# meijieru/AtomNAS

Hardware: AMD Instinct MI355X
Metric: images/sec (whole node) AtomNAS-C supernet 224x224 bs256/GPU (higher is better)
Workload: dtype bf16; 1 GPU; atomnas_c_supernet full training step (fwd + CE-smooth/L2/L1 + bwd + grad all-reduce + RMSprop + EMA), 224x224; per_gpu_batch=256, global_batch=256, parallelism=dp1, hip_graph=True

## Files before the change

atomnas_amd/csrc/pwconv.hip:

```cpp
#include "pwconv.h"

namespace atomnas {

template <typename T, int MODE, int NCG>
__global__ __launch_bounds__(256) void k_gemm_nt(Operand A, const T* __restrict__ Wp, int ldw, Epilogue ep, long M, int N, int K,
                                                 int Kpad) {
  using MM = Mma<T>;
  constexpr int E = MM::EPL;
  constexpr int KS = 4 * E;
  constexpr int SWD = 64 * NCG;
  extern __shared__ float s_stat[];

  const int tid = threadIdx.x;
  const int lane = tid & 63;
  const int wave = tid >> 6;
  const int q = lane >> 4, j = lane & 15;
  const int wrow = 16 * (j >> 2) + (j & 3);
  const bool do_stats = ep.stats != nullptr && ep.stat_mode != STAT_NONE;
  float* sw = s_stat + wave * 2 * SWD;

  if (do_stats) {
    for (int i = tid; i < 8 * SWD; i += 256) s_stat[i] = 0.f;
    __syncthreads();
  }

  const long mtiles = (M + 15) / 16;
  const int ngroups = (N + SWD - 1) / SWD;
  const int grp = blockIdx.x % ngroups, rs = blockIdx.x / ngroups, R = gridDim.x / ngroups;
  const int nc0 = grp * SWD;
  for (long mt = (long)rs * 4 + wave; mt < mtiles; mt += (long)R * 4) {
    const long m0 = mt * 16;
    const long row = m0 + j;
    const bool rowvalid = row < M;
    {
      f32x4 acc[NCG][4];
#pragma unroll
      for (int g = 0; g < NCG; ++g)
#pragma unroll
        for (int t = 0; t < 4; ++t) acc[g][t] = f32x4{0.f, 0.f, 0.f, 0.f};

#pragma unroll 2
      for (int k0 = 0; k0 < Kpad; k0 += KS) {
        const int k = k0 + q * E;
        float av[E];
        load_pro<T, MODE>(A, row, rowvalid, k, K, av);
        const typename MM::frag af = MM::pack(av);
#pragma unroll
        for (int g = 0; g < NCG; ++g) {
          const int nc = nc0 + 64 * g;
          if (nc < N) {
#pragma unroll
            for (int t = 0; t < 4; ++t) {
              const typename MM::frag wf = MM::raw(Wp + (long)(nc + wrow + 4 * t) * ldw + k);
              acc[g][t] = MM::mma(wf, af, acc[g][t]);
            }
          }
        }
      }

#pragma unroll
      for (int g = 0; g < NCG; ++g) {
        if (nc0 + 64 * g >= N) continue;
        nt_epilogue<T>(ep, acc[g], row, rowvalid, nc0 + 64 * g + 16 * q, N, do_stats, sw, SWD, 64 * g + 16 * q, j);
      }
    }
  }

  if (do_stats) nt_flush_stats(ep, s_stat, SWD, nc0, N, rs, R, tid);
}


typedef __attribute__((ext_vector_type(4))) unsigned u32x4;
typedef __attribute__((ext_vector_type(2))) unsigned u32x2;

template <int MODE, int KST, int NT = 0>
__global__ __launch_bounds__(256) void k_gemm_nt_small(Operand A, const bf16_t* __restrict__ Wp, int ldw, Epilogue ep, long M, int N, int K) {
  using T = bf16_t;
  using MM = Mma<T>;
  constexpr int SWD = 64;
  constexpr int WT = NT > 0 ? NT : 4;
  extern __shared__ float s_stat[];
  const int tid = threadIdx.x;
  const int lane = tid & 63, wave = tid >> 6;
  const int q = lane >> 4, j = lane & 15;
  const int wrow = NT > 0 ? j : 16 * (j >> 2) + (j & 3);
  const bool do_stats = ep.stats != nullptr && ep.stat_mode != STAT_NONE;
  if (do_stats) {
    for (int i = tid; i < 8 * SWD; i += 256) s_stat[i] = 0.f;
    __syncthreads();
  }
  bf16x8 wf[KST][WT];
  float p1[KST][8], p2[KST][8], p3[KST][8];
#pragma unroll
  for (int ks = 0; ks < KST; ++ks) {
    const int k = ks * 32 + 8 * q;
#pragma unroll
    for (int t = 0; t < WT; ++t) wf[ks][t] = MM::raw(Wp + (long)(wrow + (NT > 0 ? 16 : 4) * t) * ldw + k);
#pragma unroll
    for (int e = 0; e < 8; ++e) p1[ks][e] = p2[ks][e] = p3[ks][e] = 0.f;
    if constexpr (MODE != PRO_NONE) {
      if (k < K) {
        VecIO<float, 8>::load(A.c1 + k, p1[ks]);
        VecIO<float, 8>::load(A.c2 + k, p2[ks]);
        if constexpr (MODE == PRO_BNBWD) VecIO<float, 8>::load(A.c3 + k, p3[ks]);
      }
    }
  }
  struct Raw { bf16x8 a, x; };
  Raw nx[KST];
  const long mtiles = (M + 15) / 16;
  const long stride = (long)gridDim.x * 4;
  auto fetch = [&](long mt) {
    const long row = mt * 16 + j;
#pragma unroll
    for (int ks = 0; ks < KST; ++ks) {
      const int k = ks * 32 + 8 * q;
      bf16x8 z;
#pragma unroll
      for (int e = 0; e < 8; ++e) z[e] = (bf16_t)0.f;
      nx[ks].a = z;
      nx[ks].x = z;
      if (row < M && k < K) {
        nx[ks].a = *reinterpret_cast<const bf16x8*>(reinterpret_cast<const T*>(A.p1) + lay_off(row, k, A.ld1, A.ss1));
        if constexpr (MODE == PRO_BNBWD)
          nx[ks].x = *reinterpret_cast<const bf16x8*>(reinterpret_cast<const T*>(A.p2) + lay_off(row, k, A.ld2, A.ss2));
      }
    }
  };
  float s1[16], s2[16];
#pragma unroll
  for (int i = 0; i < 16; ++i) s1[i] = s2[i] = 0.f;
  float e_bias[WT][4], e_zs[WT][4], e_zh[WT][4];
  const Act e_act = act_of(ep.mask);
  if constexpr (NT > 0) {
#pragma unroll
    for (int t = 0; t < NT; ++t)
#pragma unroll
      for (int r = 0; r < 4; ++r) {
        const int n = 16 * t + 4 * q + r;
        e_bias[t][r] = (ep.bias && n < N) ? ep.bias[n] : 0.f;
        e_zs[t][r] = (ep.mask && n < N) ? ep.zscale[n] : 0.f;
        e_zh[t][r] = (ep.mask && n < N) ? ep.zshift[n] : 0.f;
      }
  }

  long mt = (long)blockIdx.x * 4 + wave;
  if (mt < mtiles) fetch(mt);
  for (; mt < mtiles; mt += stride) {
    Raw cur[KST];
#pragma unroll
    for (int ks = 0; ks < KST; ++ks) cur[ks] = nx[ks];
    if (mt + stride < mtiles) fetch(mt + stride);
    const long row = mt * 16 + j;
    const bool rowvalid = row < M;
    f32x4 acc[WT];
#pragma unroll
    for (int t = 0; t < WT; ++t) acc[t] = f32x4{0.f, 0.f, 0.f, 0.f};
#pragma unroll
    for (int ks = 0; ks < KST; ++ks) {
      const int k = ks * 32 + 8 * q;
      float v[8];
#pragma unroll
      for (int e = 0; e < 8; ++e) {
        const float a = (float)cur[ks].a[e];
        if constexpr (MODE == PRO_NONE) v[e] = a;
        else if constexpr (MODE == PRO_BNRELU) v[e] = a * p1[ks][e] + p2[ks][e];
        else v[e] = p1[ks][e] * a + p2[ks][e] * (float)cur[ks].x[e] + p3[ks][e];
      }
      if constexpr (MODE == PRO_BNRELU) act_apply_v<8>(v, act_of(A.relu));
#pragma unroll
      for (int e = 0; e < 8; ++e)
        if (!rowvalid || k + e >= K) v[e] = 0.f;
      const bf16x8 af = MM::pack(v);
#pragma unroll
      for (int t = 0; t < WT; ++t) acc[t] = MM::mma(wf[ks][t], af, acc[t]);
    }
    if constexpr (NT > 0) {
#pragma unroll
      for (int t = 0; t < NT; ++t) {
        const int c0 = 16 * t + 4 * q;
        float c[4], zv[4] = {0.f, 0.f, 0.f, 0.f};
#pragma unroll
        for (int r = 0; r < 4; ++r) c[r] = 0.f;
        if (rowvalid && c0 < N) {
#pragma unroll
          for (int r = 0; r < 4; ++r) c[r] = acc[t][r] + e_bias[t][r];
          if (ep.add) {
            const bf16x4 ad = *reinterpret_cast<const bf16x4*>(reinterpret_cast<const T*>(ep.add) + row * ep.ldadd + c0);
#pragma unroll
            for (int r = 0; r < 4; ++r) c[r] += (float)ad[r];
          }
          if (ep.z) {
            const bf16x4 zb = *reinterpret_cast<const bf16x4*>(reinterpret_cast<const T*>(ep.z) + lay_off(row, c0, ep.ldz, ep.zss));
#pragma unroll
            for (int r = 0; r < 4; ++r) zv[r] = (float)zb[r];
            if (ep.mask) {
              float a4[4];
#pragma unroll
              for (int r = 0; r < 4; ++r) a4[r] = zv[r] * e_zs[t][r] + e_zh[t][r];
              act_bwd_v<4>(c, a4, e_act);
            }
          }
          bf16x4 ob;
#pragma unroll
          for (int r = 0; r < 4; ++r) ob[r] = (bf16_t)c[r];
          u32x2 bits = __builtin_bit_cast(u32x2, ob);
          asm volatile("" : "+v"(bits));
          const f32x2 lo = bf16_pair_f32(bits[0]), hi = bf16_pair_f32(bits[1]);
          c[0] = lo[0]; c[1] = lo[1]; c[2] = hi[0]; c[3] = hi[1];
          *reinterpret_cast<u32x2*>(reinterpret_cast<T*>(ep.c) + lay_off(row, c0, ep.ldc, ep.css)) = bits;
        }
        if (do_stats) {
#pragma unroll
          for (int r = 0; r < 4; ++r) {
            s1[4 * t + r] += c[r];
            s2[4 * t + r] += (ep.stat_mode == STAT_SQ) ? c[r] * c[r] : c[r] * zv[r];
          }
        }
      }
    } else {
      float c[16], zv[16];
      nt_epilogue_core<T>(ep, acc, row, rowvalid, 16 * q, N, c, zv);
      if (do_stats) {
#pragma unroll
        for (int i = 0; i < 16; ++i) {
          s1[i] += c[i];
// ... 1391 lines not shown
    }
    ATOMNAS_RING_STAGE_END();
    islot = islot + 1 == DEPTH ? 0 : islot + 1;
    if (++ic == nchunk) { ic = 0; ++ib; }
  };

  const unsigned tr_lane = (unsigned)(((8 * q + (j >> 2)) * 16 + 4 * (j & 3)) * 2);
  auto tr_frag = [&](unsigned sub_addr) {
    const unsigned a0 = sub_addr + tr_lane;
    bf16x4 lo, hi;
    asm volatile("ds_read_b64_tr_b16 %0, %1" : "=v"(lo) : "v"(a0) : "memory");
    asm volatile("ds_read_b64_tr_b16 %0, %1 offset:128" : "=v"(hi) : "v"(a0) : "memory");
    return TrFrag{lo, hi};
  };

  f32x4 racc[NCH][UT];
#pragma unroll
  for (int c = 0; c < NCH; ++c)
#pragma unroll
    for (int t = 0; t < UT; ++t) racc[c][t] = f32x4{0.f, 0.f, 0.f, 0.f};

#pragma unroll
  for (int s = 0; s < DEPTH - 1; ++s) issue_next();
  int slot = 0;
  const unsigned row_off = (unsigned)(((wave & 1) * 16 + j) * 32);
  for (long n = 0; n < nb; ++n) {
    const long rb = rs + n * R;
    const long row = rb * 64 + wave * 16 + j;
    f32x4 acc[UT];
#pragma unroll
    for (int t = 0; t < UT; ++t) acc[t] = f32x4{0.f, 0.f, 0.f, 0.f};
    bf16x8 xa[2][UT];
#pragma unroll
    for (int c = 0; c < NCH; ++c) {
      if (c < nchunk) {
        asm volatile("s_waitcnt vmcnt(%0)" ::"n"((DEPTH - 2) * 2) : "memory");
        __syncthreads();
        issue_next();
        const unsigned base = lds_st + (unsigned)slot * STAGE_B;
        if (c == 0) {
          const unsigned xb = lds_x + (unsigned)(n & 1) * XT_B;
          TrFrag xf[2][UT];
#pragma unroll
          for (int k2 = 0; k2 < 2; ++k2)
#pragma unroll
            for (int t = 0; t < UT; ++t) xf[k2][t] = tr_frag(xb + (unsigned)(k2 * UT + t) * 1024u);
          asm volatile("s_waitcnt lgkmcnt(0)" ::: "memory");
          __builtin_amdgcn_sched_barrier(0);
#pragma unroll
          for (int k2 = 0; k2 < 2; ++k2) {
            const long rows_left = M - (rb * 64 + 32 * k2);
#pragma unroll
            for (int t = 0; t < UT; ++t) {
              xa[k2][t] = __builtin_shufflevector(xf[k2][t].lo, xf[k2][t].hi, 0, 1, 2, 3, 4, 5, 6, 7);
              if (rows_left < 32) {
#pragma unroll
                for (int e = 0; e < 8; ++e)
                  if (8 * q + e >= rows_left) xa[k2][t][e] = (bf16_t)0.f;
              }
            }
          }
        }
        TrFrag hf[2];
#pragma unroll
        for (int k2 = 0; k2 < 2; ++k2) hf[k2] = tr_frag(base + (unsigned)(4 * k2 + wave) * 1024u);
        bf16x8 hb[2];
#pragma unroll
        for (int ks = 0; ks < 2; ++ks) {
          const unsigned a = base + (unsigned)(4 * (wave >> 1) + 2 * ks + (q >> 1)) * 1024u + row_off + (unsigned)(q & 1) * 16u;
          asm volatile("ds_read_b128 %0, %1" : "=v"(hb[ks]) : "v"(a) : "memory");
        }
        asm volatile("s_waitcnt lgkmcnt(0)" ::: "memory");
        __builtin_amdgcn_sched_barrier(0);
#pragma unroll
        for (int ks = 0; ks < 2; ++ks)
#pragma unroll
          for (int t = 0; t < UT; ++t) {
            const bf16x8 wf = *reinterpret_cast<const bf16x8*>(s_w + (16 * t + j) * KP + 64 * c + 32 * ks + 8 * q);
            acc[t] = MM::mma(wf, hb[ks], acc[t]);
          }
#pragma unroll
        for (int k2 = 0; k2 < 2; ++k2) {
          const bf16x8 hv = __builtin_shufflevector(hf[k2].lo, hf[k2].hi, 0, 1, 2, 3, 4, 5, 6, 7);
#pragma unroll
          for (int t = 0; t < UT; ++t) racc[c][t] = MM::mma(xa[k2][t], hv, racc[c][t]);
        }
        slot = slot + 1 == DEPTH ? 0 : slot + 1;
      }
    }
    const unsigned xrow = lds_x + (unsigned)(n & 1) * XT_B + (unsigned)((wave >> 1) * UT) * 1024u + row_off;
    if (mpk) {
#pragma unroll
      for (int ks = 0; ks < MKS; ++ks) {
        bf16x8 xv;
#pragma unroll
        for (int e = 0; e < 8; ++e) xv[e] = (bf16_t)0.f;
        const int ct = 2 * ks + (q >> 1);
        if (ct < UT) {
          const unsigned a = xrow + (unsigned)ct * 1024u + (unsigned)(q & 1) * 16u;
          asm volatile("ds_read_b128 %0, %1\n\ts_waitcnt lgkmcnt(0)" : "=v"(xv) : "v"(a) : "memory");
        }
#pragma unroll
        for (int t = 0; t < UT; ++t) acc[t] = MM::mma(mf[ks][t], xv, acc[t]);
      }
    }
#pragma unroll
    for (int t = 0; t < UT; ++t) {
      const int c0 = 16 * t + 4 * q;
      bf16x4 av;
#pragma unroll
      for (int r = 0; r < 4; ++r) av[r] = (bf16_t)0.f;
      if (add) {
        const unsigned a = lds_a + (unsigned)(n & 1) * XT_B + (unsigned)((wave >> 1) * UT + t) * 1024u + row_off + (unsigned)(8 * q);
        asm volatile("ds_read_b64 %0, %1\n\ts_waitcnt lgkmcnt(0)" : "=v"(av) : "v"(a) : "memory");
      }
      if (row < M && c0 < N) {
        bf16x4 o;
#pragma unroll
        for (int r = 0; r < 4; ++r) o[r] = (bf16_t)(acc[t][r] + vbv[t][r] + (float)av[r]);
        *reinterpret_cast<bf16x4*>(gx + row * ldgx + c0) = o;
      }
    }
  }
  asm volatile("s_waitcnt vmcnt(0)" ::: "memory");

#pragma unroll
  for (int c = 0; c < NCH; ++c) {
    const int vc = c * 64 + 16 * wave + j;
    if (c < nchunk && vc < K) {
      const float cv = c1[vc];
#pragma unroll
      for (int t = 0; t < UT; ++t)
#pragma unroll
        for (int r = 0; r < 4; ++r) {
          const int uc = 16 * t + 4 * q + r;
          if (uc < N) ws[((long)rs * N + uc) * K + vc] = racc[c][t][r] * cv;
        }
    }
  }
}

struct NtArgs {
  int mode; Operand A;
  const void* Wp; int ldw;
  Epilogue ep;
  long M; int N, K;
  hipStream_t st;
  bool stats;
};
static NtArgs nt_args(int mode, const Operand& A, const void* Wp, int ldw, const Epilogue& ep, long M, int N, int K, hipStream_t st) {
  return NtArgs{mode, A, Wp, ldw, ep, M, N, K, st, ep.stats != nullptr && ep.stat_mode != STAT_NONE};
}

struct PwEnv { int st, sw, swg; long swg_maxm; int small_narrow, xb_stream; };
static const PwEnv& pw_env() {
  static const PwEnv e = {
      getenv("ATOMNAS_NT_ST") ? atoi(getenv("ATOMNAS_NT_ST")) : 1,
      getenv("ATOMNAS_NT_SW") ? atoi(getenv("ATOMNAS_NT_SW")) : 1,
      getenv("ATOMNAS_NT_SWG") ? atoi(getenv("ATOMNAS_NT_SWG")) : 1,
      getenv("ATOMNAS_NT_SWG_MAXM") ? atol(getenv("ATOMNAS_NT_SWG_MAXM")) : 262144,
      getenv("ATOMNAS_NT_SMALL_NARROW") ? atoi(getenv("ATOMNAS_NT_SMALL_NARROW")) : 1,
      getenv("ATOMNAS_XB_STREAM") ? atoi(getenv("ATOMNAS_XB_STREAM")) : 1,
  };
  return e;
}

template <typename KernelT>
static long row_slots(KernelT kern, int threads, size_t lds, int ngroups, long row_blocks, long cap) {
  long R = (long)num_cus() * resident_per_cu(kern, threads, lds) / ngroups;
  if (R > row_blocks) R = row_blocks;
  if (cap > 0 && R > cap) R = cap;
  return R < 1 ? 1 : R;
}
static long stat_cap(const NtArgs& a) { return a.stats ? a.ep.stat_rows : 0; }

template <typename F> static auto for_mode(int mode, F&& f) {
  if (mode == PRO_NONE) return f(IC<PRO_NONE>{});
  if (mode == PRO_BNRELU) return f(IC<PRO_BNRELU>{});
  return f(IC<PRO_BNBWD>{});
}

struct NtSwPlan { int ut, nch, depth; size_t lds; };
constexpr int SW_MAXN = 48, SW_MINK = 97, SW_MAXK = 448;
constexpr long SW_MINM = 16384;
#define SW_INSTANCES(X) X(1, 5) X(1, 7) X(2, 5) X(2, 7) X(3, 5) X(3, 7)

static bool nt_sw_plan(const NtArgs& a, NtSwPlan& p) {
  const Epilogue& ep = a.ep;
  if (!pw_env().sw || a.mode != PRO_BNRELU || a.A.ss1 <= 0 || a.N > SW_MAXN || a.N % 8 != 0 || a.K > SW_MAXK || a.K < SW_MINK ||
      a.M < SW_MINM || ep.out_f32 || ep.css != 0 || ep.add || ep.z || ep.mask || ep.bias || (a.stats && ep.stat_mode != STAT_SQ))
    return false;
  p.ut = (a.N + 15) / 16;
  p.nch = (a.K + 63) / 64 <= 5 ? 5 : 7;
  const size_t fixed = (size_t)16 * p.ut * (p.nch * 64 + 8) * sizeof(bf16_t) + (size_t)2 * p.nch * 64 * sizeof(float) +
                       (size_t)4 * 2 * 16 * p.ut * sizeof(float);
  p.depth = 2 * (fixed + 4 * 8192) + 4096 <= max_lds_bytes() ? 4 : 3;
  p.lds = fixed + (size_t)p.depth * 8192;
  return 2 * p.lds + 2048 <= max_lds_bytes();
}
template <typename KernelT>
static int nt_sw_run(const char* what, KernelT kern, int waves, size_t lds, const NtArgs& a) {
  const long R = row_slots(kern, waves * 64, lds, 1, (a.M + waves * 16 - 1) / (waves * 16), stat_cap(a));
  hipLaunchKernelGGL(kern, dim3((unsigned)R), dim3(waves * 64), lds, a.st, (const bf16_t*)a.A.p1, a.A.ss1, a.A.c1, a.A.c2, a.A.relu,
                     (const bf16_t*)a.Wp, a.ldw, (bf16_t*)a.ep.c, a.ep.ldc, a.stats ? a.ep.stats : nullptr, a.ep.stat_rows, a.M, a.N, a.K);
  return check_launch(what);
}
static int nt_sw_launch(const NtSwPlan& p, const NtArgs& a) {
#define X(UT, NCH) \
  if (p.ut == UT && p.nch == NCH) return nt_sw_run("gemm_nt_sw", p.depth == 4 ? k_gemm_nt_sw<UT, NCH, 4> : k_gemm_nt_sw<UT, NCH, 3>, 4, p.lds, a);
  SW_INSTANCES(X)
#undef X
  return 1;
}

struct NtSwgPlan { int ut; bool wide; size_t lds; };
constexpr int SWG_MAXN = 320, SWG_MINK = 256, SWG_DEPTH = 3;
constexpr long SWG_MINM = 8192;

static bool nt_swg_plan(const NtArgs& a, NtSwgPlan& p) {
  const Epilogue& ep = a.ep;
  if (!pw_env().swg || a.mode != PRO_BNRELU || a.A.ss1 <= 0 || a.N % 8 != 0 || a.N > SWG_MAXN || a.K < SWG_MINK || a.K % 4 != 0 ||
      a.M < SWG_MINM || a.M > pw_env().swg_maxm || a.ldw < 64 || a.ldw % 8 != 0 || ep.out_f32 || ep.css != 0 || ep.add || ep.z || ep.mask ||
      ep.bias || (a.stats && ep.stat_mode != STAT_SQ) || !a.A.c1 || !a.A.c2)
    return false;
  p.ut = (a.N + 15) / 16;
  if (p.ut != 3 && p.ut != 5 && p.ut != 6 && p.ut != 12 && p.ut != 20) return false;
  p.wide = (a.M + 127) / 128 >= num_cus() && p.ut <= 6;
  const int nwv = p.wide ? 8 : 4;
  p.lds = (size_t)nwv * 2 * 16 * p.ut * sizeof(float) + (size_t)SWG_DEPTH * (2 * nwv + 2 * p.ut + 1) * 1024;
  return p.lds <= max_lds_bytes();
}
static int nt_swg_launch(const NtSwgPlan& p, const NtArgs& a) {
#define X(UT, WGPC, NWV) return nt_sw_run("gemm_nt_swg", k_gemm_nt_swg<UT, SWG_DEPTH, WGPC, NWV>, NWV, p.lds, a);
  if (p.wide) {
    if (p.ut == 3) X(3, 1, 8)
    if (p.ut == 5) X(5, 1, 8)
    X(6, 1, 8)
  }
  if (p.ut == 3) X(3, 2, 4)
  if (p.ut == 5) X(5, 2, 4)
  if (p.ut == 6) X(6, 2, 4)
  if (p.ut == 12) X(12, 1, 4)
  X(20, 1, 4)
#undef X
}

struct NtStPlan { int kind, ksteps; };
constexpr int ST_MAXK = 192, ST_MINN = 96;
constexpr long ST_MINM = 1024;

static int nt_st_kind(const NtArgs& a) {
  const Operand& A = a.A;
  const Epilogue& ep = a.ep;
  const long M = a.M, N = a.N, K = a.K;
  if (!pw_env().st || a.mode != PRO_NONE || (K & 7) || ep.bias || ep.add || ep.out_f32) return 0;
  if (ep.stats != nullptr && ep.stat_mode == STAT_NONE) return 0;
  if (a.stats && ((M + 15) / 16 + ep.stat_rows - 1) / ep.stat_rows > 4096) return 0;
  const long a_bytes = A.ss1 ? ((long)((K + 15) / 16 - 1) * A.ss1 + M * 16) * 2 : M * (long)A.ld1 * 2;
  if (a_bytes >= (1L << 31)) return 0;
  if (ep.css ? (3 * ep.css + M * 16) * 2 >= (1L << 31) : ((N & 7) || (long)ep.ldc * 2 * 16 * 4096 >= (1L << 31))) return 0;
  if (!ep.z) return (!a.stats || ep.stat_mode == STAT_SQ) ? ST_FWD : 0;
  if (!ep.mask || (a.stats && ep.stat_mode != STAT_Z)) return 0;
  if (ep.zss ? (3 * ep.zss + M * 16) * 2 >= (1L << 31) : ((N & 7) || (long)ep.ldz * 2 * 16 * 4096 >= (1L << 31))) return 0;
  return ST_MASK;
}
static bool nt_st_plan(const NtArgs& a, NtStPlan& p) {
  if (a.K > ST_MAXK || a.N < 2 * a.K || a.N < ST_MINN || a.M < ST_MINM) return false;
  const int ks = (a.K + 31) / 32;
  p.ksteps = ks <= 3 ? ks : 6;
  p.kind = nt_st_kind(a);
  return p.kind != 0;
}
static long st_tiles_per_item(long mtiles, long wchunks, long waves, long min_tpi, long max_parts) {
  long tpi = (mtiles * wchunks + waves - 1) / waves;
  if (tpi < 8) tpi = 8;
  if (tpi < min_tpi) tpi = min_tpi;
  long max_ranges = waves / wchunks > 0 ? waves / wchunks : 1;
  if (max_parts > 0 && max_ranges > max_parts) max_ranges = max_parts;
  if ((mtiles + tpi - 1) / tpi > max_ranges) tpi = (mtiles + max_ranges - 1) / max_ranges;
  return tpi;
}
template <int KSTEPS, int EPK, bool SH, int BT>
static int nt_st_launch_as(const NtArgs& a) {
  using Cfg = StCfg<KSTEPS, EPK>;
  const Epilogue& ep = a.ep;
  const int nchunks = (a.N + 63) / 64;
  const long mtiles = (a.M + 15) / 16;
  const long min_tpi = ep.stats ? (mtiles + ep.stat_rows - 1) / ep.stat_rows : 1;
  auto kern = k_gemm_nt_st<KSTEPS, EPK, Cfg::PD, BT, Cfg::WPE, 0, SH>;
  const size_t lds = (size_t)(SH ? 2 : 4) * BT * KSTEPS * 1024 +
                     (EPK == ST_FWD ? 0 : (size_t)4 * (16 + 64) * PB_RP * sizeof(bf16_t) + 4 * 128 * sizeof(float));
  const long waves = (long)num_cus() * resident_per_cu(kern, 256, lds) * 4;
  const long wchunks = SH ? (long)((nchunks + 3) / 4) * 4 : nchunks;
  long tiles_per_item = st_tiles_per_item(mtiles, wchunks, waves, min_tpi, 0);
  if (tiles_per_item > 4096) tiles_per_item = 4096;
  const long nrg = (mtiles + tiles_per_item - 1) / tiles_per_item;
  const long blocks = SH ? nrg * ((nchunks + 3) / 4) : (nrg * nchunks + 3) / 4;
  hipLaunchKernelGGL(kern, dim3((unsigned)blocks), dim3(256), lds, a.st, a.A, (const bf16_t*)a.Wp, a.ldw, ep, a.M, a.N, a.K, nchunks,
                     (int)tiles_per_item, (float*)nullptr);
  return check_launch("gemm_nt_st");
}
static int nt_st_launch(const NtStPlan& p, const NtArgs& a) {
  auto go = [&](auto ks, auto epk) {
    constexpr int KSTEPS = decltype(ks)::value, EPK = decltype(epk)::value;
    using Cfg = StCfg<KSTEPS, EPK>;
    const int nchunks = (a.N + 63) / 64;
    if (Cfg::SH && ((nchunks + 3) / 4 * 4 - nchunks) * 20 <= nchunks) return nt_st_launch_as<KSTEPS, EPK, Cfg::SH, Cfg::BT>(a);
    return nt_st_launch_as<KSTEPS, EPK, false, Cfg::BTP>(a);
  };
  auto kind = [&](auto ks) { return p.kind == ST_FWD ? go(ks, IC<ST_FWD>{}) : go(ks, IC<ST_MASK>{}); };
  return p.ksteps == 1 ? kind(IC<1>{}) : p.ksteps == 2 ? kind(IC<2>{}) : p.ksteps == 3 ? kind(IC<3>{}) : kind(IC<6>{});
}

struct NtSmallPlan { int kst, ntile; };
constexpr int SMALL_MAXN = 64, SMALL_MAXK = 64;
constexpr long SMALL_MINM = 65536;

static bool nt_small_plan(const NtArgs& a, NtSmallPlan& p) {
  if (a.N > SMALL_MAXN || a.K > SMALL_MAXK || a.M < SMALL_MINM) return false;
  p.kst = a.K <= 32 ? 1 : 2;
  p.ntile = (pw_env().small_narrow && !a.ep.out_f32 && a.N % 4 == 0) ? (a.N <= 16 ? 1 : a.N <= 32 ? 2 : 4) : 0;
  return true;
}
static int nt_small_launch(const NtSmallPlan& p, const NtArgs& a) {
  auto go = [&](auto mode, auto kst) {
    constexpr int MODE = decltype(mode)::value, KST = decltype(kst)::value;
    auto kern = p.ntile == 1 ? k_gemm_nt_small<MODE, KST, 1> : p.ntile == 2 ? k_gemm_nt_small<MODE, KST, 2>
              : p.ntile == 4 ? k_gemm_nt_small<MODE, KST, 4> : k_gemm_nt_small<MODE, KST, 0>;
    const size_t lds = a.stats ? (size_t)8 * 64 * sizeof(float) : 0;
    const long R = row_slots(kern, 256, lds, 1, (a.M + 63) / 64, stat_cap(a));
    hipLaunchKernelGGL(kern, dim3((unsigned)R), dim3(256), lds, a.st, a.A, (const bf16_t*)a.Wp, a.ldw, a.ep, a.M, a.N, a.K);
  };
  for_mode(a.mode, [&](auto mode) { p.kst == 1 ? go(mode, IC<1>{}) : go(mode, IC<2>{}); });
  return check_launch("gemm_nt_small");
}

struct NtWsPlan { int ncg, rt; };
constexpr int WS_MINK = 97;
constexpr long WS_MINM = 4096;
constexpr long WS_RT2_MINM = 100000;

static bool nt_ws_plan(const NtArgs& a, NtWsPlan& p) {
  if (a.K < WS_MINK || a.M < WS_MINM) return false;
  p.ncg = a.N > 64 ? 2 : 1;
  p.rt = (a.mode == PRO_BNBWD && a.M >= WS_RT2_MINM) ? 2 : 1;
  return true;
}
template <int MODE, int NCG, int RT>
static void nt_ws_launch_as(const NtArgs& a) {
  auto kern = k_gemm_nt_ws<MODE, NCG, RT>;
  const int ngroups = (a.N + 64 * NCG - 1) / (64 * NCG);
  const size_t lds = (size_t)2 * 64 * NCG * WS_WP * sizeof(bf16_t) + 2 * 3 * WS_KC * sizeof(float) +
                     (a.stats ? (size_t)8 * 64 * NCG * sizeof(float) : 0);
  const long R = row_slots(kern, 256, lds, ngroups, (a.M + 64 * RT - 1) / (64 * RT), stat_cap(a));
  const int wrows = (a.N + 63) / 64 * 64;
  hipLaunchKernelGGL(kern, dim3((unsigned)(R * ngroups)), dim3(256), lds, a.st, a.A, (const bf16_t*)a.Wp, a.ldw, wrows, a.ep, a.M, a.N, a.K);
}
static int nt_ws_launch(const NtWsPlan& p, const NtArgs& a) {
  for_mode(a.mode, [&](auto mode) {
    constexpr int MODE = decltype(mode)::value;
    if constexpr (MODE == PRO_BNBWD) {
      if (p.rt == 2) return p.ncg == 2 ? nt_ws_launch_as<MODE, 2, 2>(a) : nt_ws_launch_as<MODE, 1, 2>(a);
    }
    return p.ncg == 2 ? nt_ws_launch_as<MODE, 2, 1>(a) : nt_ws_launch_as<MODE, 1, 1>(a);
  });
  return check_launch("gemm_nt_ws");
}

struct NtGenericPlan { int ncg; };
static bool nt_generic_plan(const NtArgs& a, NtGenericPlan& p) {
  p.ncg = a.N > 64 ? 2 : 1;
  return true;
}
template <typename T>
static int nt_generic_launch(const NtGenericPlan& p, const NtArgs& a) {
  constexpr int KS = 4 * Mma<T>::EPL;
  const int Kpad = (a.K + KS - 1) / KS * KS;
  auto go = [&](auto mode, auto ncg) {
    constexpr int NCG = decltype(ncg)::value;
    auto kern = k_gemm_nt<T, decltype(mode)::value, NCG>;
    const int ngroups = (a.N + 64 * NCG - 1) / (64 * NCG);
    const size_t lds = a.stats ? (size_t)8 * 64 * NCG * sizeof(float) : 0;
    const long R = row_slots(kern, 256, lds, ngroups, (a.M + 63) / 64, stat_cap(a));
    hipLaunchKernelGGL(kern, dim3((unsigned)(R * ngroups)), dim3(256), lds, a.st, a.A, (const T*)a.Wp, a.ldw, a.ep, a.M, a.N, a.K, Kpad);
  };
  for_mode(a.mode, [&](auto mode) { p.ncg == 2 ? go(mode, IC<2>{}) : go(mode, IC<1>{}); });
  return check_launch("gemm_nt");
}

template <typename T>
static int launch_nt(const NtArgs& a) {
  if constexpr (sizeof(T) == 2) {
    NtSwPlan sw;
    if (nt_sw_plan(a, sw)) return nt_sw_launch(sw, a);
    NtSwgPlan swg;
    if (nt_swg_plan(a, swg)) return nt_swg_launch(swg, a);
    NtStPlan st;
    if (nt_st_plan(a, st)) return nt_st_launch(st, a);
    NtSmallPlan small;
    if (nt_small_plan(a, small)) return nt_small_launch(small, a);
    NtWsPlan ws;
    if (nt_ws_plan(a, ws)) return nt_ws_launch(ws, a);
  }
  NtGenericPlan g;
  nt_generic_plan(a, g);
  return nt_generic_launch<T>(g, a);
}

static NtArgs project_bwd_args(const void* g, int ldg, const void* wpt, int ldw, const void* z, int ldz, long z_ss, const float* zscale,
                               const float* zshift, int act, void* gh, int ldgh, long gh_ss, float* stats, int stat_rows, long M, int oup,
                               int hid, hipStream_t st) {
  const Operand A{g, ldg, nullptr, 0, 0, 0, nullptr, nullptr, nullptr, 0};
  const Epilogue ep{gh, ldgh, 0, nullptr, 0, z, ldz, gh_ss, z_ss, zscale, zshift, act, nullptr, stats, STAT_Z, stat_rows};
  return nt_args(PRO_NONE, A, wpt, ldw, ep, M, hid, oup, st);
}
template <int KSTEPS, int UT>
static int launch_project_bwd_st(const NtArgs& a, float* dwp, long si, long sj, float* ws, long ws_floats) {
  using Cfg = StCfg<KSTEPS, ST_PBWD>;
  const long M = a.M;
  const int N = a.N, K = a.K;
  const int nchunks = (N + 63) / 64;
  const long mtiles = (M + 15) / 16;
  auto kern = k_gemm_nt_st<KSTEPS, ST_PBWD, Cfg::PD, Cfg::BT, Cfg::WPE, UT, false>;
  const size_t lds = (size_t)4 * Cfg::BT * KSTEPS * 1024 + (size_t)4 * (16 * UT + 64) * PB_RP * sizeof(bf16_t) + 4 * 128 * sizeof(float);
  const long waves = (long)num_cus() * resident_per_cu(kern, 256, lds) * 4;
  const long max_parts = ws_floats / ((long)K * N);
  ATOMNAS_REQUIRE(max_parts >= 1, "project_bwd: workspace too small for one partial (%ld floats)", (long)K * N);
  const long tiles_per_item = st_tiles_per_item(mtiles, nchunks, waves, (mtiles + a.ep.stat_rows - 1) / a.ep.stat_rows, max_parts);
  ATOMNAS_REQUIRE(tiles_per_item <= 4096, "project_bwd: %ld row tiles per work item (workspace / statistics rows too small for M=%ld)", tiles_per_item, M);
  const long nranges = (mtiles + tiles_per_item - 1) / tiles_per_item;
  const long items = nranges * nchunks;
  hipLaunchKernelGGL(kern, dim3((unsigned)((items + 3) / 4)), dim3(256), lds, a.st, a.A, (const bf16_t*)a.Wp, a.ldw, a.ep, M, N, K, nchunks,
                     (int)tiles_per_item, ws);
  if (int rc = check_launch("project_bwd_st")) return rc;
  return reduce_parts(ws, (long)K * N, (int)nranges, (long)K * N, dwp, N, si, sj, a.st);
}

#define XB_INSTANCES(X) X(1, 5) X(1, 7) X(1, 12) X(2, 5) X(2, 7) X(3, 5)
static inline int xb_nch(int HT) {
  const int n = (HT + WS_KC - 1) / WS_KC;
  return n <= 5 ? 5 : (n <= 7 ? 7 : (n <= 12 ? 12 : 0));
}
static bool xb_has_instance(int inp, int hid) {
  const int ut = (inp + 15) / 16, nch = xb_nch(hid);
#define X(UTV, NCHV) if (ut == UTV && nch == NCHV) return true;
  XB_INSTANCES(X)
#undef X
  return false;
}
struct XbArgs {
  const bf16_t* h; int ldh; long hss; const float* c1;
  const bf16_t* x; int ldx; const bf16_t* W; int ldw; const bf16_t* add; int ldadd; bf16_t* gx; int ldgx;
  const bf16_t* mpk; int ldm; const float* vb;
  float *dwe, *ws; long ws_floats; long M; int N, K; hipStream_t st;
};
template <typename KernelT, typename L>
static int xb_run(const char* what, const XbArgs& a, KernelT kern, size_t lds, L&& launch) {
  const long max_parts = a.ws_floats / ((long)a.N * a.K);
  ATOMNAS_REQUIRE(max_parts >= 1, "expand_bwd: workspace too small for one partial (%ld floats)", (long)a.N * a.K);
  const long R = row_slots(kern, 256, lds, 1, (a.M + 63) / 64, max_parts);
  launch((unsigned)R);
  if (int rc = check_launch(what)) return rc;
  return reduce_parts(a.ws, (long)a.N * a.K, (int)R, (long)a.N * a.K, a.dwe, a.K, 1, a.N, a.st);
}

struct XbStreamPlan { int depth; size_t lds; };
static bool xb_stream_plan(const XbArgs& a, XbStreamPlan& p) {
  if (!pw_env().xb_stream || a.hss <= 0 || a.M < 64 || a.ldx < 8 || (a.add && a.ldadd < 8)) return false;
  if ((a.K + 63) / 64 < 3) return false;
  const int ut = (a.N + 15) / 16, nch = xb_nch(a.K);
  const size_t fixed = (size_t)16 * ut * (nch * 64 + 8) * sizeof(bf16_t) + (size_t)4 * 2 * ut * 1024;
  p.depth = 2 * (fixed + 4 * 8192) + 4096 <= max_lds_bytes() ? 4 : 3;
  p.lds = fixed + (size_t)p.depth * 8192;
  return p.lds <= max_lds_bytes();
}
template <int UT, int NCH>
static int xb_stream_launch(const XbStreamPlan& p, const XbArgs& a) {
  static_assert(4 * UT * NCH <= XB_MINB2_LIMIT, "expand backward instance with too many accumulator registers");
  auto kern = p.depth == 4 ? k_expand_bwd_s<UT, NCH, 4> : k_expand_bwd_s<UT, NCH, 3>;
  return xb_run("expand_bwd(stream)", a, kern, p.lds, [&](unsigned R) {
    hipLaunchKernelGGL(kern, dim3(R), dim3(256), p.lds, a.st, a.h, a.hss, a.c1, a.W, a.ldw, a.x, a.ldx, a.add, a.ldadd, a.gx, a.ldgx, a.mpk,
                       a.ldm, a.vb, a.ws, a.M, a.N, a.K);
  });
}
template <int UT, int NCH>
static int xb_launch(const XbArgs& a) {
  static_assert(4 * UT * NCH <= XB_MINB2_LIMIT, "expand backward instance with too many accumulator registers");
  auto kern = k_expand_bwd<UT, NCH>;
  const size_t lds = (size_t)2 * 64 * WS_WP * sizeof(bf16_t) + 2 * 3 * WS_KC * sizeof(float) + (size_t)2 * 64 * XB_DP * sizeof(bf16_t) +
                     (size_t)16 * UT * XB_DP * sizeof(bf16_t);
  const Operand A{a.h, a.ldh, nullptr, 0, a.hss, 0, a.c1, a.c1, a.c1, 0};
  const Epilogue ep{a.gx, a.ldgx, 0, a.add, a.ldadd, nullptr, 0, 0, 0, nullptr, nullptr, 0, a.vb, nullptr, STAT_NONE, 0};
  const int wrows = (a.N + 63) / 64 * 64;
  return xb_run("expand_bwd", a, kern, lds, [&](unsigned R) {
    hipLaunchKernelGGL(kern, dim3(R), dim3(256), lds, a.st, A, a.W, a.ldw, wrows, a.x, a.ldx, ep, a.ws, a.M, a.N, a.K, a.mpk, a.ldm);
  });
}
static int launch_expand_bwd(const XbArgs& a) {
  const int ut = (a.N + 15) / 16, nch = xb_nch(a.K);
  XbStreamPlan sp;
  const bool stream = xb_stream_plan(a, sp);
#define X(UTV, NCHV) if (ut == UTV && nch == NCHV) return stream ? xb_stream_launch<UTV, NCHV>(sp, a) : xb_launch<UTV, NCHV>(a);
  XB_INSTANCES(X)
#undef X
  set_error("expand_bwd: no instance for inp=%d hid=%d", a.N, a.K);
  return 1;
}

}

#if WS_TIMING
extern "C" int atomnas_debug_ws_timing(unsigned long long* out8, int reset) {
  unsigned long long z[8] = {0, 0, 0, 0, 0, 0, 0, 0};
  if (out8 && hipMemcpyFromSymbol(out8, HIP_SYMBOL(atomnas::g_ws_timing), sizeof(z)) != hipSuccess) return 1;
  if (reset && hipMemcpyToSymbol(HIP_SYMBOL(atomnas::g_ws_timing), z, sizeof(z)) != hipSuccess) return 1;
  return 0;
}
#endif
using namespace atomnas;

extern "C" int atomnas_pw_gemm_nt(int a_mode, const void* a, int lda, long a_ss, const void* a2, int lda2, long a2_ss, const float* ac1,
                                  const float* ac2, const float* ac3, int a_relu, const void* wp, int ldw, void* c, int ldc, long c_ss,
                                  int out_f32, const void* add, int ldadd, const void* z, int ldz, long z_ss, const float* zscale,
                                  const float* zshift,
                                  int mask, const float* bias, float* stats, int stat_mode, int stat_rows, long M, int N, int K,
                                  int dtype, void* stream) {
  ATOMNAS_REQUIRE(dtype == DT_F32 || dtype == DT_BF16, "pw_gemm_nt: bad dtype %d", dtype);
  ATOMNAS_REQUIRE(a_mode >= PRO_NONE && a_mode <= PRO_BNBWD, "pw_gemm_nt: bad prologue %d", a_mode);
  ATOMNAS_REQUIRE(M > 0 && N > 0 && K > 0, "pw_gemm_nt: empty shape");
  ATOMNAS_REQUIRE(wp && c && (c_ss >= M * 16 || (c_ss == 0 && ldc >= N && ldc % 8 == 0)), "pw_gemm_nt: bad output/weights");
  ATOMNAS_REQUIRE(a_ss == 0 || a_ss >= M * 16, "pw_gemm_nt: slab stride of A smaller than M*16");
  {
    const int ks = (dtype == DT_BF16) ? 32 : 4;
    ATOMNAS_REQUIRE(ldw >= (K + ks - 1) / ks * ks && ldw % 8 == 0, "pw_gemm_nt: packed weight pitch %d too small for K=%d", ldw, K);
  }
  ATOMNAS_REQUIRE(!stats || N <= NT_MAX_STAT, "pw_gemm_nt: N=%d too wide for fused statistics", N);
  ATOMNAS_REQUIRE(!stats || stat_mode == STAT_NONE || stat_rows > 0, "pw_gemm_nt: statistics need stat_rows > 0");
  ATOMNAS_REQUIRE(!add || (ldadd >= N && ldadd % 8 == 0), "pw_gemm_nt: bad residual pitch");
  ATOMNAS_REQUIRE(!z || z_ss >= M * 16 || (z_ss == 0 && ldz >= N && ldz % 8 == 0), "pw_gemm_nt: bad z pitch");
  ATOMNAS_REQUIRE(!mask || (z && zscale && zshift), "pw_gemm_nt: mask needs z, zscale, zshift");
  ATOMNAS_REQUIRE(stat_mode != STAT_Z || z, "pw_gemm_nt: STAT_Z needs z");
  const Operand A{a, lda, a2, lda2, a_ss, a2_ss, ac1, ac2, ac3, a_relu};
  if (check_operand("pw_gemm_nt", A, a_mode, K)) return 1;
  const Epilogue ep{c, ldc, out_f32, add, ldadd, z, ldz, c_ss, z_ss, zscale, zshift, mask, bias, stats, stat_mode, stat_rows};
  const NtArgs args = nt_args(a_mode, A, wp, ldw, ep, M, N, K, (hipStream_t)stream);
// ... 53 lines not shown
```

atomnas_amd/csrc/pwconv_tn.hip:

```cpp
#include "pwconv.h"

namespace atomnas {

constexpr int UT_MAX = 20;
constexpr int TN_ROWS = 32;

template <typename T, int UMODE, int VMODE>
__global__ __launch_bounds__(256) void k_gemm_tn(Operand U, int NU, Operand V, int NV, float* __restrict__ out, long si, long sj,
                                                 long M, long rows_per_block, float* __restrict__ ws) {
  using MM = Mma<T>;
  constexpr int E = MM::EPL;
  constexpr int SUB = TN_ROWS / (4 * E);
  constexpr int UP = 16 * UT_MAX + 2;
  constexpr int VP = 64 + 2;
  __shared__ T s_u[TN_ROWS * UP];
  __shared__ T s_v[TN_ROWS * VP];

  const int tid = threadIdx.x;
  const int lane = tid & 63, wave = tid >> 6;
  const int q = lane >> 4, j = lane & 15;

  const int u0 = blockIdx.z * (16 * UT_MAX);
  const int nu = min(NU - u0, 16 * UT_MAX);
  const int ut = (nu + 15) / 16;
// ... 421 lines not shown
  const unsigned tr_lane = (unsigned)(((8 * q + (j >> 2)) * 16 + 4 * (j & 3)) * 2);
  auto tr_frag = [&](unsigned sub_addr) {
    const unsigned a0 = sub_addr + tr_lane;
    bf16x4 lo, hi;
    asm volatile("ds_read_b64_tr_b16 %0, %1" : "=v"(lo) : "v"(a0) : "memory");
    asm volatile("ds_read_b64_tr_b16 %0, %1 offset:128" : "=v"(hi) : "v"(a0) : "memory");
    return TrFrag{lo, hi};
  };

#pragma unroll
  for (int s = 0; s < TN3_DEPTH - 1; ++s) copy_stage(s);
  for (int s = 0; s < nstages; ++s) {
    asm volatile("s_waitcnt vmcnt(%0)" ::"n"((TN3_DEPTH - 2) * DPS) : "memory");
    __syncthreads();
    copy_stage(s + TN3_DEPTH - 1);
    const unsigned slot = lds0 + (unsigned)(s % TN3_DEPTH) * (unsigned)(STAGE * 2);
    TrFrag bfp[2], afp[UTT];
#pragma unroll
    for (int v = 0; v < 2; ++v) bfp[v] = tr_frag(slot + (unsigned)(4 * v + wave) * 1024u);
#pragma unroll
    for (int t = 0; t < UTT; ++t)
      if (t < ut) afp[t] = tr_frag(slot + (unsigned)(8 + t) * 1024u);
    asm volatile("s_waitcnt lgkmcnt(0)" ::: "memory");
    __builtin_amdgcn_sched_barrier(0);
    bf16x8 bf[2];
#pragma unroll
    for (int v = 0; v < 2; ++v) {
      bf[v] = __builtin_shufflevector(bfp[v].lo, bfp[v].hi, 0, 1, 2, 3, 4, 5, 6, 7);
      if constexpr (VPRO) {
        float x[8];
#pragma unroll
        for (int e = 0; e < 8; ++e) x[e] = (float)bf[v][e] * vsc[v] + vsh[v];
        act_apply_v<8>(x, vact);
        bf[v] = MM::pack(x);
      }
    }
    const long rows_left = r_end - (r_beg + 32L * s);
#pragma unroll
    for (int t = 0; t < UTT; ++t) {
      if (t < ut) {
        bf16x8 af = __builtin_shufflevector(afp[t].lo, afp[t].hi, 0, 1, 2, 3, 4, 5, 6, 7);
        if (rows_left < 32) {
#pragma unroll
          for (int e = 0; e < 8; ++e)
            if (8 * q + e >= rows_left) af[e] = (bf16_t)0.f;
        }
#pragma unroll
        for (int v = 0; v < 2; ++v) acc[v][t] = MM::mma(af, bf[v], acc[v][t]);
      }
    }
  }
  asm volatile("s_waitcnt vmcnt(0)" ::: "memory");

#pragma unroll
  for (int v = 0; v < 2; ++v) {
    const int vc = v0 + 64 * v + 16 * wave + j;
    if (vc < NV) {
#pragma unroll
      for (int t = 0; t < UTT; ++t) {
        if (t < ut) {
#pragma unroll
          for (int r = 0; r < 4; ++r) {
            const int uc = u0 + 16 * t + 4 * q + r;
            if (uc < NU) {
              if (ws) ws[(chunk * NU + uc) * NV + vc] = acc[v][t][r];
              else out[uc * si + vc * sj] += acc[v][t][r];
            }
          }
        }
      }
    }
  }
}

struct TnArgs {
  int umode; Operand U; int NU;
  int vmode; Operand V; int NV;
  float* out; long si, sj, M;
  float* ws; long ws_floats;
  hipStream_t st;
};

template <int... Vs, typename F> static int for_value(int v, F&& f) {
  int rc = 1;
  (void)((v == Vs ? (rc = f(IC<Vs>{}), true) : false) || ...);
  return rc;
}
template <typename F> static int for_pair(int umode, int vmode, F&& f) {
#define X(UM, VM) if (umode == UM && vmode == VM) return f(IC<UM>{}, IC<VM>{});
  X(PRO_NONE, PRO_NONE) X(PRO_NONE, PRO_BNBWD) X(PRO_BNBWD, PRO_BNRELU) X(PRO_BNRELU, PRO_BNBWD) X(PRO_BNBWD, PRO_NONE)
  X(PRO_NONE, PRO_BNRELU)
#undef X
  set_error("gemm_tn: unsupported prologue pair (%d,%d)", umode, vmode);
  return 1;
}

static int tn_utt(int NU, bool dma) {
  const int ut = (NU + 15) / 16;
  return ut <= 2 ? (dma ? 4 : 2) : ut <= 4 ? 4 : ut <= 6 ? 6 : ut <= 12 ? 12 : ut <= 20 ? 10 : 20;
}

static long tn_ws_cap(const TnArgs& a) { return a.ws ? a.ws_floats / ((long)a.NU * a.NV) : 1; }
static void tn_split(long M, long want, long min_rows, long quantum, long& chunks, long& rows) {
  if (want < 1) want = 1;
  rows = (M + want - 1) / want;
  if (rows < min_rows) rows = min_rows;
  rows = (rows + quantum - 1) / quantum * quantum;
  chunks = (M + rows - 1) / rows;
}
static int tn_finish(const char* what, const TnArgs& a, long chunks) {
  if (int rc = check_launch(what)) return rc;
  if (chunks > 1) return reduce_parts(a.ws, (long)a.NU * a.NV, (int)chunks, (long)a.NU * a.NV, a.out, a.NV, a.si, a.sj, a.st);
  return 0;
}

using TnDmaKernel = decltype(&k_gemm_tn3<4, false, 4>);
struct TnDmaPlan { TnDmaKernel kern; int utt, vt, uz; size_t lds; long chunks, rows; unsigned grid; };
constexpr int DMA_MINNU = 32, DMA_MINNV = 256;
constexpr long DMA_MINM = 1024, DMA_MINROWS = 128;
constexpr int tn3_depth(int utt) { return 2 * (4 * (8 + utt) * 1024) + 4096 <= 160 * 1024 ? 4 : 3; }
static bool tn_dma_plan(const TnArgs& a, TnDmaPlan& p) {
  static const int on = getenv("ATOMNAS_TN_DMA") ? atoi(getenv("ATOMNAS_TN_DMA")) : 1;
  if (!on || a.umode != PRO_NONE || (a.vmode != PRO_NONE && a.vmode != PRO_BNRELU) || !a.ws) return false;
  if (a.NV < DMA_MINNV || a.NU < DMA_MINNU || a.M < DMA_MINM) return false;
  p.utt = tn_utt(a.NU, true);
  if (for_value<4, 6, 12, 10>(p.utt, [&](auto utt) {
        constexpr int UTT = decltype(utt)::value, DEPTH = tn3_depth(UTT);
        p.kern = a.vmode == PRO_BNRELU ? k_gemm_tn3<UTT, true, DEPTH> : k_gemm_tn3<UTT, false, DEPTH>;
        p.lds = (size_t)DEPTH * (8 + UTT) * 1024;
        return 0;
      }))
    return false;
  if (p.lds > max_lds_bytes()) return false;
  p.vt = (a.NV + 127) / 128, p.uz = (a.NU + 16 * p.utt - 1) / (16 * p.utt);
  const long tiles = (long)p.vt * p.uz;
  long want = (long)num_cus() * resident_per_cu(p.kern, 256, p.lds) / tiles;
  if (want > a.M / DMA_MINROWS) want = a.M / DMA_MINROWS;
  if (want > tn_ws_cap(a)) want = tn_ws_cap(a);
  want = want / 8 * 8;
  if (want < 8) return false;
  tn_split(a.M, want, 0, 32, p.chunks, p.rows);
  p.grid = (unsigned)((p.chunks + 7) / 8 * 8 * tiles);
  return true;
}
static int tn_dma_launch(const TnDmaPlan& p, const TnArgs& a) {
  hipLaunchKernelGGL(p.kern, dim3(p.grid), dim3(256), p.lds, a.st, a.U, a.NU, a.V, a.NV, a.out, a.si, a.sj, a.M, p.rows, (int)p.chunks, p.vt,
                     p.uz, a.ws);
  return tn_finish("gemm_tn3", a, p.chunks);
}

using TnSlabKernel = decltype(&k_gemm_tn2<PRO_NONE, PRO_NONE, 2, 1, 128>);
struct TnSlabPlan { TnSlabKernel kern; int utt, vtt, slab_rows, vt, uz; size_t lds; long chunks, rows; int xcd; unsigned grid; };
constexpr int SLAB_WIDE_MINNV = 256;
static bool tn_slab_plan(const TnArgs& a, TnSlabPlan& p) {
  p.utt = tn_utt(a.NU, false);
  const bool wide = p.utt >= 4 && p.utt <= 12 && a.NV >= SLAB_WIDE_MINNV;
  p.vtt = wide ? 2 : 1, p.slab_rows = wide ? 64 : 128;
  if (for_pair(a.umode, a.vmode, [&](auto um, auto vm) {
        return for_value<2, 4, 6, 12, 10, 20>(p.utt, [&](auto utt) {
          constexpr int UM = decltype(um)::value, VM = decltype(vm)::value, UTT = decltype(utt)::value;
          p.kern = k_gemm_tn2<UM, VM, UTT, 1, 128>;
          if constexpr (UTT >= 4 && UTT <= 12)
            if (wide) p.kern = k_gemm_tn2<UM, VM, UTT, 2, 64>;
          return 0;
        });
      }))
    return false;
  const int vw = 64 * p.vtt, uw = 16 * p.utt;
  p.vt = (a.NV + vw - 1) / vw, p.uz = (a.NU + uw - 1) / uw;
  p.lds = (size_t)(vw + uw) * (p.slab_rows + 8) * sizeof(bf16_t) + (size_t)3 * (vw + uw) * sizeof(float);
  const long tiles = (long)p.vt * p.uz;
  long want = (long)num_cus() * resident_per_cu(p.kern, 256, p.lds) / tiles;
  if (want > a.M / (2 * p.slab_rows)) want = a.M / (2 * p.slab_rows);
  if (want > tn_ws_cap(a)) want = tn_ws_cap(a);
  p.xcd = want >= 8;
  if (p.xcd) want = want / 8 * 8;
  tn_split(a.M, want, 0, 1, p.chunks, p.rows);
  p.grid = (unsigned)((p.xcd ? (p.chunks + 7) / 8 * 8 : p.chunks) * tiles);
  return true;
}
static int tn_slab_launch(const TnSlabPlan& p, const TnArgs& a) {
  hipLaunchKernelGGL(p.kern, dim3(p.grid), dim3(256), p.lds, a.st, a.U, a.NU, a.V, a.NV, a.out, a.si, a.sj, a.M, p.rows, (int)p.chunks, p.vt,
                     p.uz, p.xcd, p.chunks > 1 ? a.ws : nullptr);
  return tn_finish("gemm_tn2", a, p.chunks);
}

using TnGenericKernel = decltype(&k_gemm_tn<float, PRO_NONE, PRO_NONE>);
struct TnGenericPlan { TnGenericKernel kern; int vt, uz; long chunks, rows; };
static bool tn_generic_plan(const TnArgs& a, TnGenericPlan& p) {
  if (for_pair(a.umode, a.vmode, [&](auto um, auto vm) { p.kern = k_gemm_tn<float, decltype(um)::value, decltype(vm)::value>; return 0; }))
    return false;
  p.vt = (a.NV + 63) / 64, p.uz = (a.NU + 16 * UT_MAX - 1) / (16 * UT_MAX);
  const long tiles = (long)p.vt * p.uz;
  long want = (1024 + tiles - 1) / tiles;
  if (want > tn_ws_cap(a)) want = tn_ws_cap(a);
  tn_split(a.M, want, 8 * TN_ROWS, TN_ROWS, p.chunks, p.rows);
  return true;
}
static int tn_generic_launch(const TnGenericPlan& p, const TnArgs& a) {
  hipLaunchKernelGGL(p.kern, dim3((unsigned)p.chunks, p.vt, p.uz), dim3(256), 0, a.st, a.U, a.NU, a.V, a.NV, a.out, a.si, a.sj, a.M, p.rows,
                     p.chunks > 1 ? a.ws : nullptr);
  return tn_finish("gemm_tn", a, p.chunks);
}

static int launch_tn(const TnArgs& a, int dtype) {
  TnDmaPlan dma; TnSlabPlan slab; TnGenericPlan generic;
  if (dtype == DT_BF16 && tn_dma_plan(a, dma)) return tn_dma_launch(dma, a);
  if (dtype == DT_BF16 && tn_slab_plan(a, slab)) return tn_slab_launch(slab, a);
  if (dtype == DT_F32 && tn_generic_plan(a, generic)) return tn_generic_launch(generic, a);
  return 1;
}

}

using namespace atomnas;

extern "C" int atomnas_pw_gemm_tn(int u_mode, const void* u, int ldu, long u_ss, const void* u2, int ldu2, long u2_ss, const float* uc1,
                                  const float* uc2, const float* uc3, int u_relu, int NU, int v_mode, const void* v, int ldv, long v_ss,
                                  const void* v2, int ldv2, long v2_ss, const float* vc1, const float* vc2, const float* vc3, int v_relu, int NV, float* out,
                                  long si, long sj, long M, float* ws, long ws_floats, int dtype, void* stream) {
  ATOMNAS_REQUIRE(dtype == DT_F32 || dtype == DT_BF16, "pw_gemm_tn: bad dtype %d", dtype);
  ATOMNAS_REQUIRE(M > 0 && NU > 0 && NV > 0 && out, "pw_gemm_tn: empty shape");
  Operand U{u, ldu, u2, ldu2, u_ss, u2_ss, uc1, uc2, uc3, u_relu};
  Operand V{v, ldv, v2, ldv2, v_ss, v2_ss, vc1, vc2, vc3, v_relu};
  ATOMNAS_REQUIRE((u_ss == 0 || u_ss >= M * 16) && (v_ss == 0 || v_ss >= M * 16), "pw_gemm_tn: slab stride smaller than M*16");
  if (check_operand("pw_gemm_tn(U)", U, u_mode, NU)) return 1;
  if (check_operand("pw_gemm_tn(V)", V, v_mode, NV)) return 1;
  return launch_tn(TnArgs{u_mode, U, NU, v_mode, V, NV, out, si, sj, M, ws, ws_floats, (hipStream_t)stream}, dtype);
}
```

Measured before the change: 9629 images/sec.

## Add few-row NT GEMM kernel, wider WS column groups, and finer TN slab tiling

```diff
diff --git a/atomnas_amd/csrc/pwconv.hip b/atomnas_amd/csrc/pwconv.hip
--- a/atomnas_amd/csrc/pwconv.hip
+++ b/atomnas_amd/csrc/pwconv.hip
@@ -72,6 +72,76 @@
 
 typedef __attribute__((ext_vector_type(4))) unsigned u32x4;
 typedef __attribute__((ext_vector_type(2))) unsigned u32x2;
+
+constexpr int FEW_U = 8;
+template <bool OUT_F32>
+__global__ __launch_bounds__(256) void k_gemm_nt_few(const bf16_t* __restrict__ A, int lda, const bf16_t* __restrict__ Wp, int ldw,
+                                                     void* __restrict__ cout, int ldc, const float* __restrict__ bias, int M, int N, int K) {
+  using MM = Mma<bf16_t>;
+  const int lane = threadIdx.x & 63;
+  const int q = lane >> 4, j = lane & 15;
+  const int wave = __builtin_amdgcn_readfirstlane((int)(threadIdx.x >> 6));
+  const int ntm = (M + 15) / 16, ntn = (N + 15) / 16;
+  const int tile = blockIdx.x * 4 + wave;
+  if (tile >= ntm * ntn) return;
+  const int m0 = (tile % ntm) * 16, n0 = (tile / ntm) * 16;
+  const int row = m0 + j;
+  const bool rowvalid = row < M;
+  const int ksteps = (K + 31) / 32;
+  const int K8 = (K + 7) & ~7;
+  const bf16_t* ap = A + (long)(rowvalid ? row : M - 1) * lda;
+  const bf16_t* wp = Wp + (long)(n0 + j) * ldw;
+
+  auto fetch = [&](int s0, bf16x8 (&a)[FEW_U], bf16x8 (&w)[FEW_U]) {
+#pragma unroll
+    for (int u = 0; u < FEW_U; ++u) {
+      const int k = (s0 + u) * 32 + 8 * q;
+      a[u] = *reinterpret_cast<const bf16x8*>(ap + (k < K ? k : K8 - 8));
+      w[u] = *reinterpret_cast<const bf16x8*>(wp + (s0 + u < ksteps ? k : 8 * q));
+    }
+  };
+  f32x4 acc = f32x4{0.f, 0.f, 0.f, 0.f};
+  auto mac = [&](int s0, const bf16x8 (&a)[FEW_U], const bf16x8 (&w)[FEW_U]) {
+#pragma unroll
+    for (int u = 0; u < FEW_U; ++u) {
+      if (s0 + u < ksteps) {
+        const int k = (s0 + u) * 32 + 8 * q;
+        bf16x8 af = a[u];
+#pragma unroll
+        for (int e = 0; e < 8; ++e)
+          if (!rowvalid || k + e >= K) af[e] = (bf16_t)0.f;
+        acc = MM::mma(w[u], af, acc);
+      }
+    }
+  };
+  bf16x8 a0[FEW_U], w0[FEW_U], a1[FEW_U], w1[FEW_U];
+  fetch(0, a0, w0);
+  for (int s = 0; s < ksteps; s += 2 * FEW_U) {
+    fetch(s + FEW_U, a1, w1);
+    mac(s, a0, w0);
+    fetch(s + 2 * FEW_U, a0, w0);
+    mac(s + FEW_U, a1, w1);
+  }
+
+  const int c0 = n0 + 4 * q;
+  if (rowvalid && (c0 & ~7) < N) {
+    float c[4];
+#pragma unroll
+    for (int r = 0; r < 4; ++r) {
+      c[r] = acc[r];
+      if (bias) c[r] += (c0 + r < N) ? bias[c0 + r] : 0.f;
+      if (c0 + r >= N) c[r] = 0.f;
+    }
+    if constexpr (OUT_F32) {
+      *reinterpret_cast<f32x4*>(reinterpret_cast<float*>(cout) + (long)row * ldc + c0) = f32x4{c[0], c[1], c[2], c[3]};
+    } else {
+      bf16x4 o;
+#pragma unroll
+      for (int r = 0; r < 4; ++r) o[r] = (bf16_t)c[r];
+      *reinterpret_cast<bf16x4*>(reinterpret_cast<bf16_t*>(cout) + (long)row * ldc + c0) = o;
+    }
+  }
+}
 
 template <int MODE, int KST, int NT = 0>
 __global__ __launch_bounds__(256) void k_gemm_nt_small(Operand A, const bf16_t* __restrict__ Wp, int ldw, Epilogue ep, long M, int N, int K) {
@@ -1769,7 +1839,7 @@
   return NtArgs{mode, A, Wp, ldw, ep, M, N, K, st, ep.stats != nullptr && ep.stat_mode != STAT_NONE};
 }
 
-struct PwEnv { int st, sw, swg; long swg_maxm; int small_narrow, xb_stream; };
+struct PwEnv { int st, sw, swg; long swg_maxm; int small_narrow, xb_stream, ws_wide, few; };
 static const PwEnv& pw_env() {
   static const PwEnv e = {
       getenv("ATOMNAS_NT_ST") ? atoi(getenv("ATOMNAS_NT_ST")) : 1,
@@ -1778,6 +1848,8 @@
       getenv("ATOMNAS_NT_SWG_MAXM") ? atol(getenv("ATOMNAS_NT_SWG_MAXM")) : 262144,
       getenv("ATOMNAS_NT_SMALL_NARROW") ? atoi(getenv("ATOMNAS_NT_SMALL_NARROW")) : 1,
       getenv("ATOMNAS_XB_STREAM") ? atoi(getenv("ATOMNAS_XB_STREAM")) : 1,
+      getenv("ATOMNAS_NT_WS_WIDE") ? atoi(getenv("ATOMNAS_NT_WS_WIDE")) : 1,
+      getenv("ATOMNAS_NT_FEW") ? atoi(getenv("ATOMNAS_NT_FEW")) : 1,
   };
   return e;
 }
@@ -1795,6 +1867,25 @@
   if (mode == PRO_NONE) return f(IC<PRO_NONE>{});
   if (mode == PRO_BNRELU) return f(IC<PRO_BNRELU>{});
   return f(IC<PRO_BNBWD>{});
+}
+
+struct NtFewPlan { bool f32; };
+constexpr long FEW_MAXM = 512;
+constexpr int FEW_MINK = 512;
+static bool nt_few_plan(const NtArgs& a, NtFewPlan& p) {
+  const Epilogue& ep = a.ep;
+  if (!pw_env().few || a.mode != PRO_NONE || a.M > FEW_MAXM || a.K < FEW_MINK || a.A.ss1 != 0 || ep.css != 0 || ep.add || ep.z || ep.mask ||
+      a.stats)
+    return false;
+  p.f32 = ep.out_f32 != 0;
+  return true;
+}
+static int nt_few_launch(const NtFewPlan& p, const NtArgs& a) {
+  const long tiles = ((a.M + 15) / 16) * ((a.N + 15) / 16);
+  auto kern = p.f32 ? k_gemm_nt_few<true> : k_gemm_nt_few<false>;
+  hipLaunchKernelGGL(kern, dim3((unsigned)((tiles + 3) / 4)), dim3(256), 0, a.st, (const bf16_t*)a.A.p1, a.A.ld1, (const bf16_t*)a.Wp, a.ldw,
+                     a.ep.c, a.ep.ldc, a.ep.bias, (int)a.M, a.N, a.K);
+  return check_launch("gemm_nt_few");
 }
 
 struct NtSwPlan { int ut, nch, depth; size_t lds; };
@@ -1957,10 +2048,12 @@
 constexpr long WS_MINM = 4096;
 constexpr long WS_RT2_MINM = 100000;
 
+constexpr int WS_WIDE_MAXN = 192;
 static bool nt_ws_plan(const NtArgs& a, NtWsPlan& p) {
   if (a.K < WS_MINK || a.M < WS_MINM) return false;
   p.ncg = a.N > 64 ? 2 : 1;
   p.rt = (a.mode == PRO_BNBWD && a.M >= WS_RT2_MINM) ? 2 : 1;
+  if (pw_env().ws_wide && a.mode == PRO_BNBWD && !a.stats && a.N > 128 && a.N <= WS_WIDE_MAXN && p.rt == 1) p.ncg = 3;
   return true;
 }
 template <int MODE, int NCG, int RT>
@@ -1978,6 +2071,7 @@
     constexpr int MODE = decltype(mode)::value;
     if constexpr (MODE == PRO_BNBWD) {
       if (p.rt == 2) return p.ncg == 2 ? nt_ws_launch_as<MODE, 2, 2>(a) : nt_ws_launch_as<MODE, 1, 2>(a);
+      if (p.ncg == 3) return nt_ws_launch_as<MODE, 3, 1>(a);
     }
     return p.ncg == 2 ? nt_ws_launch_as<MODE, 2, 1>(a) : nt_ws_launch_as<MODE, 1, 1>(a);
   });
@@ -2008,6 +2102,8 @@
 template <typename T>
 static int launch_nt(const NtArgs& a) {
   if constexpr (sizeof(T) == 2) {
+    NtFewPlan few;
+    if (nt_few_plan(a, few)) return nt_few_launch(few, a);
     NtSwPlan sw;
     if (nt_sw_plan(a, sw)) return nt_sw_launch(sw, a);
     NtSwgPlan swg;
diff --git a/atomnas_amd/csrc/pwconv_tn.hip b/atomnas_amd/csrc/pwconv_tn.hip
--- a/atomnas_amd/csrc/pwconv_tn.hip
+++ b/atomnas_amd/csrc/pwconv_tn.hip
@@ -597,10 +597,9 @@
 using TnSlabKernel = decltype(&k_gemm_tn2<PRO_NONE, PRO_NONE, 2, 1, 128>);
 struct TnSlabPlan { TnSlabKernel kern; int utt, vtt, slab_rows, vt, uz; size_t lds; long chunks, rows; int xcd; unsigned grid; };
 constexpr int SLAB_WIDE_MINNV = 256;
-static bool tn_slab_plan(const TnArgs& a, TnSlabPlan& p) {
-  p.utt = tn_utt(a.NU, false);
-  const bool wide = p.utt >= 4 && p.utt <= 12 && a.NV >= SLAB_WIDE_MINNV;
-  p.vtt = wide ? 2 : 1, p.slab_rows = wide ? 64 : 128;
+constexpr long SLAB_FEW_MAXM = 512;
+static bool tn_slab_instance(const TnArgs& a, TnSlabPlan& p) {
+  const bool wide = p.vtt == 2;
   if (for_pair(a.umode, a.vmode, [&](auto um, auto vm) {
         return for_value<2, 4, 6, 12, 10, 20>(p.utt, [&](auto utt) {
           constexpr int UM = decltype(um)::value, VM = decltype(vm)::value, UTT = decltype(utt)::value;
@@ -614,6 +613,13 @@
   const int vw = 64 * p.vtt, uw = 16 * p.utt;
   p.vt = (a.NV + vw - 1) / vw, p.uz = (a.NU + uw - 1) / uw;
   p.lds = (size_t)(vw + uw) * (p.slab_rows + 8) * sizeof(bf16_t) + (size_t)3 * (vw + uw) * sizeof(float);
+  return true;
+}
+static bool tn_slab_plan(const TnArgs& a, TnSlabPlan& p) {
+  p.utt = tn_utt(a.NU, false);
+  const bool wide = p.utt >= 4 && p.utt <= 12 && a.NV >= SLAB_WIDE_MINNV;
+  p.vtt = wide ? 2 : 1, p.slab_rows = wide ? 64 : 128;
+  if (!tn_slab_instance(a, p)) return false;
   const long tiles = (long)p.vt * p.uz;
   long want = (long)num_cus() * resident_per_cu(p.kern, 256, p.lds) / tiles;
   if (want > a.M / (2 * p.slab_rows)) want = a.M / (2 * p.slab_rows);
@@ -622,6 +628,19 @@
   if (p.xcd) want = want / 8 * 8;
   tn_split(a.M, want, 0, 1, p.chunks, p.rows);
   p.grid = (unsigned)((p.xcd ? (p.chunks + 7) / 8 * 8 : p.chunks) * tiles);
+  static const int few = getenv("ATOMNAS_NT_FEW") ? atoi(getenv("ATOMNAS_NT_FEW")) : 1;
+  if (few && a.M <= SLAB_FEW_MAXM && p.chunks == 1) {
+    const int cand_wide[] = {12, 6, 4}, cand_plain[] = {20, 12, 10, 6, 4, 2};
+    const int* cand = wide ? cand_wide : cand_plain;
+    const int ncand = wide ? 3 : 6, first = p.utt;
+    for (int i = 0; i < ncand; ++i) {
+      if (cand[i] > first) continue;
+      p.utt = cand[i];
+      if ((long)p.vt * ((a.NU + 16 * p.utt - 1) / (16 * p.utt)) >= num_cus()) break;
+    }
+    if (p.utt != first && !tn_slab_instance(a, p)) return false;
+    p.grid = (unsigned)((long)p.vt * p.uz);
+  }
   return true;
 }
 static int tn_slab_launch(const TnSlabPlan& p, const TnArgs& a) {
```

Result: no change. 9671 images/sec, median of 6 (+0.4%).
